# Alexander-H-Liu/End-to-end-ASR-Pytorch

Hardware: NVIDIA H100
Metric: utterances/sec (train step, ~12s@16kHz synthetic) (higher is better)
Workload: dtype f32

## Files before the change

end-to-end-asr-pytorch_b200/csrc/gemm.cu:

```cuda
#include <cuda.h>
#include <cuda_fp16.h>
#include <stdlib.h>
#include "common.cuh"
#include "wgmma.cuh"
#include "../../include/b200asr.h"

namespace b200asr {
namespace {

constexpr int G_BM = 128, G_BN = 128, G_BK = 32;
constexpr int G_TILE = G_BM * G_BK * 4;
constexpr int G_CONSUMERS = 256;
constexpr int G_THREADS = 128 + G_CONSUMERS;
constexpr int G_PREP_WARPS = 3;
constexpr int G_PRODUCER_REGS = 40, G_CONSUMER_REGS = 232;
constexpr int G_BOX = 32 * G_BK * 4;
constexpr int G_MAX_SPLIT = 32;
constexpr int G_CH_DEFAULT = 4;

template <bool B_MN>
struct GemmSmem {
    static constexpr int STAGE = (B_MN ? 4 : 3) * G_TILE;
    static constexpr int STAGES = B_MN ? 3 : 4;
    static constexpr int B_LO = 2 * G_TILE;
// ... 417 lines not shown

struct F16Args {
    const float* bias;
    const float* sa;
    const float* sb;
    float* C;
    float* partial;
    int M, N, ldc, accumulate, perm;
    int KB, kb_per_split;
};

__device__ __forceinline__ int f16_scale_exp(uint32_t amax) {
    if (amax == 0u || amax >= 0x7f800000u) return 0;
    const int E = amax >= 0x00800000u ? (int)(amax >> 23) - 127 : (31 - __clz((int)amax)) - 149;
    return min(126, max(-126, 13 - E));
}
__device__ __forceinline__ float pow2f(int e) { return __uint_as_float((uint32_t)(127 + e) << 23); }
__device__ __forceinline__ uint32_t abs_bits(float x) { return __float_as_uint(x) & 0x7fffffffu; }
__device__ __forceinline__ void f16_split2(float x0, float x1, float s, __half2& hi, __half2& lo) {
    const float y0 = x0 * s, y1 = x1 * s;
    hi = __floats2half2_rn(y0, y1);
    lo = __floats2half2_rn(y0 - __low2float(hi), y1 - __high2float(hi));
}

__global__ void __launch_bounds__(256) f16_split_rows_kernel(const float* __restrict__ x, long long ld, int rows, int K,
                                                             int Kp, __half* __restrict__ hi, __half* __restrict__ lo,
                                                             float* __restrict__ sinv) {
    const int row = blockIdx.x * 8 + (threadIdx.x >> 5), lane = threadIdx.x & 31, c = blockIdx.y;
    if (row >= rows) return;
    const int k = c * F_CK + 4 * lane;
    float4 v = make_float4(0.f, 0.f, 0.f, 0.f);
    if (k < K) v = *reinterpret_cast<const float4*>(x + (size_t)row * ld + k);
    const uint32_t a = __reduce_max_sync(0xffffffffu, max(max(abs_bits(v.x), abs_bits(v.y)), max(abs_bits(v.z), abs_bits(v.w))));
    const int e = f16_scale_exp(a);
    const float s = pow2f(e);
    __half2 h[2], l[2];
    f16_split2(v.x, v.y, s, h[0], l[0]);
    f16_split2(v.z, v.w, s, h[1], l[1]);
    const size_t o = (size_t)row * Kp + k;
    *reinterpret_cast<uint2*>(hi + o) = *reinterpret_cast<const uint2*>(h);
    *reinterpret_cast<uint2*>(lo + o) = *reinterpret_cast<const uint2*>(l);
    if (lane == 0) sinv[(size_t)c * rows + row] = pow2f(-e);
}

__global__ void __launch_bounds__(256) f16_split_cols_kernel(const float* __restrict__ x, long long ld, long long bstride,
                                                             int shift, int T, int R, int cols, int Rp,
                                                             __half* __restrict__ hi, __half* __restrict__ lo,
                                                             float* __restrict__ sinv) {
    __shared__ float tile[F_CK][65];
    const int r0 = blockIdx.y * F_CK, c0 = blockIdx.x * 64, tid = threadIdx.x;
    const int cq = 4 * (tid & 15);
#pragma unroll
    for (int i = 0; i < F_CK / 16; ++i) {
        const int rr = (tid >> 4) + 16 * i, r = r0 + rr;
        float4 v = make_float4(0.f, 0.f, 0.f, 0.f);
        if (r < R && c0 + cq < cols) {
            const int b = r / T, t = r - b * T + shift;
            if (t >= 0 && t < T) v = *reinterpret_cast<const float4*>(x + b * bstride + (long long)t * ld + c0 + cq);
        }
        tile[rr][cq] = v.x; tile[rr][cq + 1] = v.y; tile[rr][cq + 2] = v.z; tile[rr][cq + 3] = v.w;
    }
    __syncthreads();
    const int warp = tid >> 5, lane = tid & 31;
    for (int j = 0; j < 8; ++j) {
        const int cc = 8 * warp + j, col = c0 + cc;
        if (col >= cols) break;
        const float v0 = tile[2 * lane][cc], v1 = tile[2 * lane + 1][cc];
        const float v2 = tile[64 + 2 * lane][cc], v3 = tile[65 + 2 * lane][cc];
        const uint32_t a = __reduce_max_sync(0xffffffffu, max(max(abs_bits(v0), abs_bits(v1)), max(abs_bits(v2), abs_bits(v3))));
        const int e = f16_scale_exp(a);
        const float s = pow2f(e);
        __half2 h0, l0, h1, l1;
        f16_split2(v0, v1, s, h0, l0);
        f16_split2(v2, v3, s, h1, l1);
        const size_t o = (size_t)col * Rp + r0 + 2 * lane;
        *reinterpret_cast<__half2*>(hi + o) = h0;
        *reinterpret_cast<__half2*>(hi + o + 64) = h1;
        *reinterpret_cast<__half2*>(lo + o) = l0;
        *reinterpret_cast<__half2*>(lo + o + 64) = l1;
        if (lane == 0) sinv[(size_t)blockIdx.y * cols + col] = pow2f(-e);
    }
}

__device__ __forceinline__ void f16_chunk(float (&d)[64], int i0, const uint8_t* smem, uint64_t* full, uint64_t* empty,
                                          uint32_t a_off, int lane) {
#pragma unroll
    for (int j = 0; j < F_CH; ++j) {
        const int i = i0 + j, s = i % F_STAGES;
        mbar_wait(&full[s], (uint32_t)((i / F_STAGES) & 1));
        const uint32_t st = smem_u32(smem + s * F_STAGE);
        const uint32_t ahi = st + a_off, alo = ahi + F_TILE, bhi = st + 2 * F_TILE, blo = st + 3 * F_TILE;
        wgmma::fence_operand(d);
        wgmma::fence();
#pragma unroll
        for (int k = 0; k < F_BK / 16; ++k) {
            const uint64_t dah = wgmma::desc_k_sw128(ahi + 32 * k), dbh = wgmma::desc_k_sw128(bhi + 32 * k);
            wgmma::mma_f16_n128(d, dah, dbh, (j | k) != 0);
            wgmma::mma_f16_n128(d, dah, wgmma::desc_k_sw128(blo + 32 * k), 1);
            wgmma::mma_f16_n128(d, wgmma::desc_k_sw128(alo + 32 * k), dbh, 1);
        }
        wgmma::commit_group();
        if (j + 1 < F_CH) wgmma::wait_group<1>();
        else wgmma::wait_all();
        if (lane == 0 && j > 0) g_arrive(&empty[(i - 1) % F_STAGES]);
    }
    wgmma::fence_operand(d);
    if (lane == 0) g_arrive(&empty[(i0 + F_CH - 1) % F_STAGES]);
}

__global__ void __launch_bounds__(G_THREADS, 1)
gemm_f16x3_kernel(const __grid_constant__ CUtensorMap map_ahi, const __grid_constant__ CUtensorMap map_alo,
                  const __grid_constant__ CUtensorMap map_bhi, const __grid_constant__ CUtensorMap map_blo,
                  const F16Args g) {
    extern __shared__ __align__(1024) uint8_t smem[];
    uint64_t* full = reinterpret_cast<uint64_t*>(smem + F_STAGES * F_STAGE);
    uint64_t* empty = full + F_STAGES;
    const int tid = threadIdx.x, warp = tid >> 5, lane = tid & 31;
    const int m0 = blockIdx.y * G_BM, n0 = blockIdx.x * G_BN;
    const int kb0 = blockIdx.z * g.kb_per_split;
    auto slice_blocks = [&]() { return min(g.KB, kb0 + g.kb_per_split) - kb0; };
    if (tid == 0) {
        for (int s = 0; s < F_STAGES; ++s) {
            mbar_init(&full[s], 1);
            mbar_init(&empty[s], G_CONSUMERS / 32);
        }
        mbar_fence_init();
    }
    __syncthreads();

    if (warp < 4) {
        asm volatile("setmaxnreg.dec.sync.aligned.u32 %0;" ::"n"(G_PRODUCER_REGS) : "memory");
        if (warp == 0 && lane == 0) {
            const int nkb = slice_blocks();
            for (int i = 0; i < nkb; ++i) {
                const int s = i % F_STAGES, k = (kb0 + i) * F_BK;
                if (i >= F_STAGES) mbar_wait(&empty[s], (uint32_t)(((i / F_STAGES) - 1) & 1));
                uint8_t* st = smem + s * F_STAGE;
                mbar_expect_tx(&full[s], 4 * F_TILE);
                tma_load_2d(st, &map_ahi, k, m0, &full[s]);
                tma_load_2d(st + F_TILE, &map_alo, k, m0, &full[s]);
                tma_load_2d(st + 2 * F_TILE, &map_bhi, k, n0, &full[s]);
                tma_load_2d(st + 3 * F_TILE, &map_blo, k, n0, &full[s]);
            }
        }
    } else {
        asm volatile("setmaxnreg.inc.sync.aligned.u32 %0;" ::"n"(G_CONSUMER_REGS) : "memory");
        const int nkb = slice_blocks();
        const int wg = (warp >> 2) - 1;
        const int r0 = 64 * wg + 16 * (warp & 3) + (lane >> 2);
        const int row0 = m0 + r0, row1 = row0 + 8;
        const int M = g.M, N = g.N;
        float acc[64], d[64];
#pragma unroll
        for (int e = 0; e < 64; ++e) acc[e] = 0.f;
        for (int i = 0; i < nkb; i += F_CH) {
            const size_t c = (size_t)((kb0 + i) / F_CH);
            const float sa0 = row0 < M ? g.sa[c * M + row0] : 0.f, sa1 = row1 < M ? g.sa[c * M + row1] : 0.f;
            float sb[32];
#pragma unroll
            for (int gq = 0; gq < 16; ++gq) {
                const int n = n0 + 8 * gq + 2 * (lane & 3);
                sb[2 * gq] = n < N ? g.sb[c * N + n] : 0.f;
                sb[2 * gq + 1] = n + 1 < N ? g.sb[c * N + n + 1] : 0.f;
            }
            f16_chunk(d, i, smem, full, empty, (uint32_t)(wg * 64 * 128), lane);
#pragma unroll
// ... 64 lines not shown
}

extern "C" int b200asr_gemm3x_nn(const float* A, int lda, const float* B, int ldb, const float* bias, float* C, int M,
                                 int N, int K, int ldc, int accumulate, void* workspace, size_t workspace_bytes,
                                 b200asr_stream stream) {
    B200_REQUIRE(A && B && C, "gemm3x_nn: null pointer");
    B200_REQUIRE(M > 0 && N > 0 && K > 0, "gemm3x_nn: bad sizes M=%d N=%d K=%d", M, N, K);
    B200_REQUIRE(lda >= K && (lda % 4) == 0 && ldb >= N && (ldb % 4) == 0 && ldc >= N,
                 "gemm3x_nn: row pitches must be multiples of 4 floats (lda %d ldb %d ldc %d)", lda, ldb, ldc);
    B200_REQUIRE(aligned16(A) && aligned16(B), "gemm3x_nn: operands must be 16-byte aligned");
    CUtensorMap ma, mb;
    int rc = make_map_k(&ma, A, M, K, lda, G_BM);
    if (rc != B200_OK) return rc;
    rc = make_map_mn(&mb, B, N, K, 1, ldb, 0, false);
    if (rc != B200_OK) return rc;
    GemmArgs g = {};
    g.bias = bias; g.C = C; g.M = M; g.N = N; g.ldc = ldc; g.accumulate = accumulate;
    g.KB = (K + G_BK - 1) / G_BK; g.kbt = g.KB;
    return launch<false, true>(ma, mb, g, workspace, workspace_bytes, (cudaStream_t)stream);
}

extern "C" int b200asr_gemm3x_nt(const float* A, long long lda, long long a_bstride, int a_shift, const float* B,
                                 long long ldb, long long b_bstride, int b_shift, float* C, int M, int N, int T,
                                 int batches, int ldc, int accumulate, int permute_rows, void* workspace,
                                 size_t workspace_bytes, b200asr_stream stream) {
    B200_REQUIRE(A && B && C, "gemm3x_nt: null pointer");
    B200_REQUIRE(M > 0 && N > 0 && T > 0 && batches > 0, "gemm3x_nt: bad sizes M=%d N=%d T=%d batches=%d", M, N, T,
                 batches);
    B200_REQUIRE(lda > 0 && (lda % 4) == 0 && ldb > 0 && (ldb % 4) == 0 && (a_bstride % 4) == 0 &&
                     (b_bstride % 4) == 0 && ldc >= N,
                 "gemm3x_nt: pitches must be multiples of 4 floats (lda %lld ldb %lld)", lda, ldb);
    B200_REQUIRE(aligned16(A) && aligned16(B), "gemm3x_nt: operands must be 16-byte aligned");
    B200_REQUIRE(!permute_rows || (M % 4) == 0, "gemm3x_nt: the row permutation needs M %% 4 == 0");
    B200_REQUIRE(a_shift >= -G_BK && a_shift <= G_BK && b_shift >= -G_BK && b_shift <= G_BK, "gemm3x_nt: bad shift");
    CUtensorMap ma, mb;
    int rc = make_map_mn(&ma, A, M, T, batches, lda, a_bstride, true);
    if (rc != B200_OK) return rc;
    rc = make_map_mn(&mb, B, N, T, batches, ldb, b_bstride, false);
    if (rc != B200_OK) return rc;
    GemmArgs g = {};
    g.C = C; g.M = M; g.N = N; g.ldc = ldc; g.accumulate = accumulate; g.perm = permute_rows;
    g.kbt = (T + G_BK - 1) / G_BK; g.KB = g.kbt * batches;
    g.a_shift = a_shift; g.b_shift = b_shift;
    return launch<true, true>(ma, mb, g, workspace, workspace_bytes, (cudaStream_t)stream);
}

extern "C" int b200asr_tf32_residual(const float* x, float* lo, long long n, b200asr_stream stream) {
    B200_REQUIRE(x && lo && n >= 0, "tf32_residual: bad arguments");
    if (n == 0) return B200_OK;
    const long long per_block = 256LL * RES_UNROLL * 4;
    tf32_residual_kernel<<<(unsigned)((n + per_block - 1) / per_block), 256, 0, (cudaStream_t)stream>>>(x, lo, n);
    B200_LAUNCH_CHECK("tf32_residual_kernel");
    return B200_OK;
}

extern "C" int b200asr_f16x3_padded_k(int K) { return K > 0 ? (K + F_CK - 1) / F_CK * F_CK : 0; }

extern "C" int b200asr_f16x3_split_rows(const float* x, long long ld, int rows, int K, void* hi, void* lo, float* sinv,
                                        b200asr_stream stream) {
    B200_REQUIRE(x && hi && lo && sinv, "f16x3_split_rows: null pointer");
    B200_REQUIRE(rows > 0 && K > 0 && (K % 4) == 0 && ld >= K && (ld % 4) == 0 && aligned16(x),
                 "f16x3_split_rows: needs K %% 4 == 0, a pitch that is a multiple of 4 floats, 16-byte alignment "
                 "(rows %d K %d ld %lld)", rows, K, ld);
    const int Kp = b200asr_f16x3_padded_k(K);
    dim3 grid((rows + 7) / 8, Kp / F_CK);
    f16_split_rows_kernel<<<grid, 256, 0, (cudaStream_t)stream>>>(x, ld, rows, K, Kp, (__half*)hi, (__half*)lo, sinv);
    B200_LAUNCH_CHECK("f16_split_rows_kernel");
    return B200_OK;
}

extern "C" int b200asr_f16x3_split_cols(const float* x, long long ld, long long bstride, int shift, int T, int batches,
                                        int cols, void* hi, void* lo, float* sinv, b200asr_stream stream) {
    B200_REQUIRE(x && hi && lo && sinv, "f16x3_split_cols: null pointer");
    B200_REQUIRE(T > 0 && batches > 0 && cols > 0 && (cols % 4) == 0 && ld >= cols && (ld % 4) == 0 &&
                     (bstride % 4) == 0 && (batches == 1 || bstride >= (long long)T * ld) && aligned16(x),
                 "f16x3_split_cols: needs cols %% 4 == 0, pitches that are multiples of 4 floats, 16-byte alignment "
                 "(cols %d ld %lld bstride %lld)", cols, ld, bstride);
    B200_REQUIRE((long long)T * batches < (1LL << 31) - F_CK, "f16x3_split_cols: too many rows");
    const int R = T * batches, Rp = b200asr_f16x3_padded_k(R);
    dim3 grid((cols + 63) / 64, Rp / F_CK);
    f16_split_cols_kernel<<<grid, 256, 0, (cudaStream_t)stream>>>(x, ld, bstride, shift, T, R, cols, Rp, (__half*)hi,
                                                                  (__half*)lo, sinv);
    B200_LAUNCH_CHECK("f16_split_cols_kernel");
    return B200_OK;
}

extern "C" int b200asr_gemm_f16x3(const void* a_hi, const void* a_lo, const float* a_sinv, const void* b_hi,
                                  const void* b_lo, const float* b_sinv, const float* bias, float* C, int M, int N,
                                  int Kp, int ldc, int accumulate, int permute_rows, void* workspace,
                                  size_t workspace_bytes, b200asr_stream stream) {
    B200_REQUIRE(a_hi && a_lo && a_sinv && b_hi && b_lo && b_sinv && C, "gemm_f16x3: null pointer");
    B200_REQUIRE(M > 0 && N > 0 && Kp > 0 && (Kp % F_CK) == 0 && ldc >= N,
                 "gemm_f16x3: bad sizes M=%d N=%d Kp=%d ldc=%d (Kp must be b200asr_f16x3_padded_k of K)", M, N, Kp, ldc);
    B200_REQUIRE(aligned16(a_hi) && aligned16(a_lo) && aligned16(b_hi) && aligned16(b_lo),
                 "gemm_f16x3: images must be 16-byte aligned");
    B200_REQUIRE(!permute_rows || (M % 4) == 0, "gemm_f16x3: the row permutation needs M %% 4 == 0");
    CUtensorMap mah, mal, mbh, mbl;
    int rc;
    if ((rc = make_map_f16(&mah, a_hi, M, Kp)) != B200_OK) return rc;
    if ((rc = make_map_f16(&mal, a_lo, M, Kp)) != B200_OK) return rc;
    if ((rc = make_map_f16(&mbh, b_hi, N, Kp)) != B200_OK) return rc;
    if ((rc = make_map_f16(&mbl, b_lo, N, Kp)) != B200_OK) return rc;
    F16Args g = {};
    g.bias = bias; g.sa = a_sinv; g.sb = b_sinv; g.C = C;
    g.M = M; g.N = N; g.ldc = ldc; g.accumulate = accumulate; g.perm = permute_rows;
    g.KB = Kp / F_BK;
    int nsplit = pick_split(M, N, Kp / G_BK);
    if (nsplit > 1 && (workspace == nullptr || workspace_bytes < (size_t)nsplit * M * N * sizeof(float))) nsplit = 1;
    const int chunks = g.KB / F_CH;
    g.kb_per_split = (chunks + nsplit - 1) / nsplit * F_CH;
    nsplit = (g.KB + g.kb_per_split - 1) / g.kb_per_split;
    g.partial = reinterpret_cast<float*>(workspace);
    const size_t smem = (size_t)F_STAGES * F_STAGE + 256;
    cudaStream_t st = (cudaStream_t)stream;
    B200_CUDA(cudaFuncSetAttribute(gemm_f16x3_kernel, cudaFuncAttributeMaxDynamicSharedMemorySize, (int)smem));
    dim3 grid((N + G_BN - 1) / G_BN, (M + G_BM - 1) / G_BM, nsplit);
    gemm_f16x3_kernel<<<grid, G_THREADS, smem, st>>>(mah, mal, mbh, mbl, g);
    B200_LAUNCH_CHECK("gemm_f16x3_kernel");
    if (nsplit > 1) {
        const long long total = (long long)M * N;
        int blocks = (int)((total + 255) / 256);
        if (blocks > 16 * sm_count()) blocks = 16 * sm_count();
        gemm3x_reduce_kernel<<<blocks, 256, 0, st>>>(g.partial, nsplit, bias, C, M, N, ldc, accumulate, permute_rows);
        B200_LAUNCH_CHECK("gemm3x_reduce_kernel");
    }
    return B200_OK;
}
```

end-to-end-asr-pytorch_b200/lib.py:

```python
import ctypes
import os
from ctypes import c_int, c_float, c_longlong, c_size_t, c_void_p, c_char_p, c_ulonglong, POINTER

import torch

_HERE = os.path.dirname(os.path.abspath(__file__))
LIB_PATH = os.path.join(_HERE, "libb200asr.so")

_lib = None

_P = c_void_p
SIGNATURES = {
    "b200asr_version": (c_int, []),
    "b200asr_last_error": (c_char_p, []),
    "b200asr_launch_count": (c_ulonglong, []),
    "b200asr_launch_count_reset": (None, []),
    "b200asr_device_sm_count": (c_int, []),
    "b200asr_fbank_fwd": (c_int, [_P, _P, c_int, c_int, c_int, c_int, c_int, c_float, c_int, _P, c_int, _P, _P, _P, _P,
                                  c_int, c_int, c_float, _P, c_int, _P, _P]),
    "b200asr_fbank_fwd_pcm16": (c_int, [_P, _P, c_int, c_int, c_int, c_int, c_int, c_float, c_int, _P, c_int, _P, _P, _P, _P,
                                  c_int, c_int, c_float, _P, c_int, _P, _P]),
    "b200asr_delta_cmvn_workspace_bytes": (c_size_t, [c_int, c_int, c_int, c_int]),
    "b200asr_delta_cmvn_fwd": (c_int, [_P, _P, c_int, c_int, c_int, c_int, c_int, c_int, c_float, _P, _P, c_size_t,
                                       _P]),
    "b200asr_log_softmax_fwd": (c_int, [_P, _P, _P, _P, c_longlong, c_int, _P]),
    "b200asr_log_softmax_bwd": (c_int, [_P, _P, _P, c_longlong, c_int, _P]),
    "b200asr_ctc_workspace_bytes": (c_size_t, [c_int, c_int, c_int]),
    "b200asr_ctc_fwd_bwd": (c_int, [_P, c_longlong, c_longlong, _P, _P, _P, c_int, c_int, c_int, c_int, c_int, _P, _P,
                                    _P, _P, c_size_t, _P]),
    "b200asr_ctc_grad": (c_int, [_P, c_longlong, c_longlong, _P, _P, _P, c_int, c_int, c_int, c_int, c_int, _P, _P, _P,
                                 _P, _P, c_size_t, _P]),
    "b200asr_ctc_fwd_bwd_logits": (c_int, [_P, _P, c_longlong, c_longlong, _P, _P, _P, c_int, c_int, c_int, c_int, c_int, _P,
                                           _P, _P, _P, c_size_t, _P]),
    "b200asr_ctc_grad_logits": (c_int, [_P, _P, c_longlong, c_longlong, _P, _P, _P, c_int, c_int, c_int, c_int, c_int, _P,
                                        _P, _P, _P, _P, c_size_t, _P]),
    "b200asr_ctc_prefix_score": (c_int, [_P, c_int, c_int, _P, _P, _P, _P, c_int, c_int, c_int, c_int, _P, _P, _P]),
    "b200asr_bilstm_workspace_bytes": (c_size_t, [c_int, c_int, c_int, c_int]),
    "b200asr_bilstm_plan": (c_int, [c_int, c_int, c_int, POINTER(c_int), POINTER(c_int), POINTER(c_int)]),
    "b200asr_bilstm_uses_tensor_cores": (c_int, [c_int, c_int, c_int]),
    "b200asr_bilstm_uses_tcgen05": (c_int, [c_int, c_int, c_int]),
    "b200asr_bilstm_fwd": (c_int, [_P, _P, _P, _P, c_int, c_int, c_int, c_int, _P, c_size_t, _P]),
    "b200asr_bilstm_bwd": (c_int, [_P, _P, _P, _P, c_int, c_int, c_int, c_int, _P, c_size_t, _P]),
    "b200asr_debug_set_lstm_trace": (None, [_P]),
    "b200asr_debug_set_lstm_mode": (None, [c_int]),
    "b200asr_debug_lstm_variant": (c_int, [c_int, c_int, c_int, c_int, POINTER(c_int)]),
    "b200asr_debug_ctc_variant": (c_int, [c_int]),
    "b200asr_debug_locattn_bwd_minb": (c_int, [c_int, c_int, c_int, c_int]),
    "b200asr_lstm_cell_fwd": (c_int, [_P, _P, _P, _P, _P, c_int, c_int, _P]),
    "b200asr_lstm_cell_bwd": (c_int, [_P, _P, _P, _P, _P, _P, _P, c_int, c_int, _P]),
    "b200asr_locattn_cluster_size": (c_int, [c_int, c_int]),
    "b200asr_locattn_wpart_floats": (c_size_t, [c_int, c_int, c_int]),
    "b200asr_locattn_fwd": (c_int, [_P, _P, _P, _P, _P, _P, _P, _P, _P, c_float, c_int, c_int, c_int, c_int, c_int,
                                    c_int, _P, _P, _P]),
    "b200asr_locattn_bwd": (c_int, [_P, _P, _P, _P, _P, _P, _P, _P, c_float, _P, _P, _P, c_int, c_int, c_int, c_int,
                                    c_int, c_int, _P, _P, _P, _P, _P, _P]),
    "b200asr_locattn_bwd_acc": (c_int, [_P, _P, _P, _P, _P, _P, _P, _P, c_float, _P, _P, _P, c_int, c_int, c_int, c_int,
                                        c_int, c_int, _P, _P, _P, _P, _P]),
    "b200asr_attn_dvalue": (c_int, [_P, _P, c_int, c_int, c_int, c_int, _P, c_int, _P]),
    "b200asr_ce_fwd_bwd": (c_int, [_P, _P, c_longlong, c_longlong, c_int, _P, _P, _P, _P]),
    "b200asr_embedding_bwd_workspace_bytes": (c_size_t, [c_int, c_int]),
    "b200asr_embedding_bwd": (c_int, [_P, _P, c_int, c_int, c_int, _P, _P, c_size_t, _P]),
    "b200asr_gemm3x_tn": (c_int, [_P, c_int, _P, _P, _P, _P, c_int, c_int, c_int, c_int, c_int, _P, c_size_t, _P]),
    "b200asr_gemm3x_nn": (c_int, [_P, c_int, _P, c_int, _P, _P, c_int, c_int, c_int, c_int, c_int, _P, c_size_t, _P]),
    "b200asr_gemm3x_workspace_bytes": (c_size_t, [c_int, c_int]),
    "b200asr_gemm3x_nt": (c_int, [_P, c_longlong, c_longlong, c_int, _P, c_longlong, c_longlong, c_int, _P, c_int, c_int,
                                  c_int, c_int, c_int, c_int, c_int, _P, c_size_t, _P]),
    "b200asr_tf32_residual": (c_int, [_P, _P, c_longlong, _P]),
    "b200asr_f16x3_padded_k": (c_int, [c_int]),
    "b200asr_f16x3_split_rows": (c_int, [_P, c_longlong, c_int, c_int, _P, _P, _P, _P]),
    "b200asr_f16x3_split_cols": (c_int, [_P, c_longlong, c_longlong, c_int, c_int, c_int, c_int, _P, _P, _P, _P]),
    "b200asr_gemm_f16x3": (c_int, [_P, _P, _P, _P, _P, _P, _P, _P, c_int, c_int, c_int, c_int, c_int, c_int, _P, c_size_t,
                                   _P]),
    "b200asr_split_tf32": (c_int, [_P, _P, _P, c_longlong, _P]),
    "b200asr_grad_norm_scratch_bytes": (c_size_t, []),
    "b200asr_grad_norm": (c_int, [_P, c_longlong, _P, _P, _P]),
    "b200asr_adadelta_step": (c_int, [_P, _P, _P, _P, c_longlong, c_float, c_float, c_float, c_float, _P, c_float, _P]),
    "b200asr_adam_step": (c_int, [_P, _P, _P, _P, c_longlong, c_float, c_float, c_float, c_float, c_float, c_int, _P,
                                  c_float, _P]),
}


class B200AsrError(RuntimeError):
    pass


def load(build_if_missing=False):
    global _lib
    if _lib is not None:
        return _lib
    if not os.path.exists(LIB_PATH):
        if build_if_missing:
            from . import _build
            _build.build()
        else:
            raise B200AsrError(
                "libb200asr.so is missing (%s): run `python -c 'import __graft_entry__ as g; g.build()'`; "
                "there is no CPU fallback" % LIB_PATH)
    lib = ctypes.CDLL(LIB_PATH)
    for name, (res, args) in SIGNATURES.items():
        fn = getattr(lib, name)
        fn.restype = res
        fn.argtypes = args
    _lib = lib
    return lib


def last_error():
    return load().b200asr_last_error().decode("utf-8", "replace")


def check(rc, what=""):
    if rc != 0:
        raise B200AsrError("%s failed (rc=%d): %s" % (what or "b200asr call", rc, last_error()))


def ptr(t):
    if t is None:
        return None
    if not t.is_cuda:
        raise B200AsrError("b200asr kernels need CUDA tensors (got a %s tensor); there is no CPU fallback" % t.device)
    return c_void_p(t.data_ptr())


def stream():
    return c_void_p(torch.cuda.current_stream().cuda_stream)


def launch_count():
    return int(load().b200asr_launch_count())


def launch_count_reset():
    load().b200asr_launch_count_reset()


class KernelTimer:

    def __init__(self):
        self.enabled = False
        self.records = []

    def reset(self):
        self.records = []

    def summary(self):
        out = {}
        for name, a, b, nbytes in self.records:
            d = out.setdefault(name, {"launches": 0, "ms": 0.0, "bytes": 0})
            d["launches"] += 1
            d["ms"] += a.elapsed_time(b)
            d["bytes"] += nbytes
        return out

# ... 21 lines not shown
```

end-to-end-asr-pytorch_b200/ops.py:

```python
import ctypes
import os

import torch
from torch.autograd import Function

from . import lib as L


def _f32c(t):
    if t.dtype != torch.float32:
        raise L.B200AsrError("b200asr kernels compute in fp32 (got %s)" % t.dtype)
    return t if t.is_contiguous() else t.contiguous()


def _gemm_exact():
    torch.backends.cuda.matmul.allow_tf32 = False
    torch.backends.cudnn.allow_tf32 = False


_gemm_exact()

_perm_cache = {}


# ... 29 lines not shown
    b = _f32c(bias) if bias is not None else None
    ws, ws_bytes = None, 0
    if w_lo is not None or M <= 256:
        ws_bytes = lib.b200asr_gemm3x_workspace_bytes(M, N)
        ws = torch.empty(max(ws_bytes, 16), device=a.device, dtype=torch.uint8)
    with L.timed("gemm3x_tn", 4 * (M * K + N * K + M * N * (2 if accumulate else 1))):
        L.check(lib.b200asr_gemm3x_tn(L.ptr(a), K, L.ptr(w), L.ptr(w_lo), L.ptr(b), L.ptr(out), M, N, K, out.stride(0),
                                      int(bool(accumulate)), L.ptr(ws), ws_bytes, L.stream()), "gemm3x_tn")
    return out


def gemm_tn_ld(a_base, lda, M, K, w, bias=None):
    lib = L.load()
    w = _f32c(w)
    N = w.shape[0]
    out = torch.empty((M, N), device=w.device, dtype=torch.float32)
    b = _f32c(bias) if bias is not None else None
    with L.timed("gemm3x_tn", 4 * (M * lda + N * K + M * N)):
        L.check(lib.b200asr_gemm3x_tn(L.ptr(a_base), lda, L.ptr(w), None, L.ptr(b), L.ptr(out), M, N, K, N, 0, None, 0,
                                      L.stream()), "gemm3x_tn")
    return out


def gemm_nn(a, w, out=None, accumulate=False):
    lib = L.load()
    a, w = _f32c(a), _f32c(w)
    M, K = a.shape
    N = w.shape[1]
    if out is None:
        out = torch.empty((M, N), device=a.device, dtype=torch.float32)
        accumulate = False
    assert out.stride(1) == 1 and out.shape == (M, N)
    ws, ws_bytes = None, 0
    if M <= 256:
        ws_bytes = lib.b200asr_gemm3x_workspace_bytes(M, N)
        ws = torch.empty(max(ws_bytes, 16), device=a.device, dtype=torch.uint8)
    with L.timed("gemm3x_nn", 4 * (M * K + N * K + M * N * (2 if accumulate else 1))):
        L.check(lib.b200asr_gemm3x_nn(L.ptr(a), K, L.ptr(w), N, None, L.ptr(out), M, N, K, out.stride(0),
                                      int(bool(accumulate)), L.ptr(ws), ws_bytes, L.stream()), "gemm3x_nn")
    return out


def gemm_nt(a, b, M, N, T, batches=1, lda=None, a_bstride=0, ldb=None, b_bstride=0, b_shift=0, permute_rows=False,
            out=None, accumulate=False):
    lib = L.load()
    lda = M if lda is None else lda
    ldb = N if ldb is None else ldb
    if out is None:
        out = torch.empty((M, N), device=a.device, dtype=torch.float32)
        accumulate = False
    assert out.is_contiguous() and out.dtype == torch.float32 and out.numel() == M * N
    ws_bytes = lib.b200asr_gemm3x_workspace_bytes(M, N)
    ws = torch.empty(max(ws_bytes, 16), device=a.device, dtype=torch.uint8)
    with L.timed("gemm3x_nt", 4 * (batches * T * (M + N) + M * N * (2 if accumulate else 1))):
        L.check(lib.b200asr_gemm3x_nt(L.ptr(a), lda, a_bstride, 0, L.ptr(b), ldb, b_bstride, b_shift, L.ptr(out), M, N,
                                      T, batches, N, int(bool(accumulate)), int(bool(permute_rows)), L.ptr(ws),
                                      ws_bytes, L.stream()),
                "gemm3x_nt")
    return out


def f16_split(x, rows, K, ld=None):
    lib = L.load()
    ld = K if ld is None else ld
    Kp = lib.b200asr_f16x3_padded_k(K)
    img = torch.empty((2, rows, Kp), device=x.device, dtype=torch.float16)
    sinv = torch.empty((Kp // 128, rows), device=x.device, dtype=torch.float32)
    with L.timed("f16_split", 4 * rows * K + 4 * rows * Kp):
        L.check(lib.b200asr_f16x3_split_rows(L.ptr(x), ld, rows, K, L.ptr(img[0]), L.ptr(img[1]), L.ptr(sinv),
                                             L.stream()), "f16x3_split_rows")
    return img, sinv


def f16_split_t(x, cols, T, batches=1, ld=None, bstride=0, shift=0):
    lib = L.load()
    ld = cols if ld is None else ld
    Rp = lib.b200asr_f16x3_padded_k(batches * T)
    img = torch.empty((2, cols, Rp), device=x.device, dtype=torch.float16)
    sinv = torch.empty((Rp // 128, cols), device=x.device, dtype=torch.float32)
    with L.timed("f16_split", 4 * batches * T * cols + 4 * cols * Rp):
        L.check(lib.b200asr_f16x3_split_cols(L.ptr(x), ld, bstride, shift, T, batches, cols, L.ptr(img[0]),
                                             L.ptr(img[1]), L.ptr(sinv), L.stream()), "f16x3_split_cols")
    return img, sinv


def gemm_f16x3(a, b, bias=None, out=None, accumulate=False, permute_rows=False, name="gemm_f16_tn"):
    lib = L.load()
    (aimg, asinv), (bimg, bsinv) = a, b
    M, Kp = aimg.shape[1], aimg.shape[2]
    N = bimg.shape[1]
    assert bimg.shape[2] == Kp
    if out is None:
        out = torch.empty((M, N), device=aimg.device, dtype=torch.float32)
        accumulate = False
    assert out.dtype == torch.float32 and out.stride(1) == 1 and out.shape == (M, N)
    ws_bytes = lib.b200asr_gemm3x_workspace_bytes(M, N)
    ws = torch.empty(max(ws_bytes, 16), device=aimg.device, dtype=torch.uint8)
    bb = _f32c(bias) if bias is not None else None
    with L.timed(name, 4 * Kp * (M + N) + 4 * M * N * (2 if accumulate else 1)):
        L.check(lib.b200asr_gemm_f16x3(L.ptr(aimg[0]), L.ptr(aimg[1]), L.ptr(asinv), L.ptr(bimg[0]), L.ptr(bimg[1]),
                                       L.ptr(bsinv), L.ptr(bb), L.ptr(out), M, N, Kp, out.stride(0),
                                       int(bool(accumulate)), int(bool(permute_rows)), L.ptr(ws), ws_bytes,
                                       L.stream()), "gemm_f16x3")
    return out


class Conv1dK4S2Fn(Function):

    @staticmethod
    def forward(ctx, x, weight, bias):
        x = _f32c(x)
        B, T, C = x.shape
        O = weight.shape[0]
        Tout = T // 2
        Tp = 2 * (Tout + 1)
        xp = torch.zeros((B, Tp, C), device=x.device, dtype=torch.float32)
        xp[:, 1:T + 1] = x
        wm = weight.detach().permute(0, 2, 1).reshape(O, 4 * C).contiguous()
        M = B * (Tp // 2) - 1
        yf = torch.empty((B * (Tp // 2), O), device=x.device, dtype=torch.float32)
        yf[M:] = 0
        yf[:M] = gemm_tn_ld(xp, 2 * C, M, 4 * C, wm, bias.detach() if bias is not None else None)
        ctx.save_for_backward(xp, wm)
        ctx.dims = (B, T, C, O, Tout, Tp, M)
        ctx.has_bias = bias is not None
        return yf.view(B, Tp // 2, O)[:, :Tout]

    @staticmethod
    def backward(ctx, dy):
        xp, wm = ctx.saved_tensors
        B, T, C, O, Tout, Tp, M = ctx.dims
        half = Tp // 2
        dyf = torch.zeros((B, half, O), device=dy.device, dtype=torch.float32)
        dyf[:, :Tout] = dy
        dy2 = dyf.view(B * half, O)
        dx = None
        if ctx.needs_input_grad[0]:
            dcols = gemm_nn(dy2, wm).view(B, half, 2, 2 * C)
            dxp = torch.zeros((B, half + 1, 2 * C), device=dy.device, dtype=torch.float32)
            dxp[:, :half] += dcols[:, :, 0]
            dxp[:, 1:] += dcols[:, :, 1]
            dx = dxp.view(B, Tp + 2, C)[:, 1:T + 1].contiguous()
        dw = db = None
        if ctx.needs_input_grad[1]:
            dwm = gemm_nt(dy2, xp, O, 4 * C, M, ldb=2 * C)
            dw = dwm.view(O, 4, C).permute(0, 2, 1).contiguous()
        if ctx.has_bias and ctx.needs_input_grad[2]:
            db = dy.reshape(-1, O).sum(0)
        return dx, dw, db


def conv1d_k4s2p1(x, conv):
    C = x.shape[-1]
    if (x.is_cuda and conv.kernel_size == (4,) and conv.stride == (2,) and conv.padding == (1,) and x.shape[1] >= 2
            and (2 * C) % 4 == 0):
        return Conv1dK4S2Fn.apply(x, conv.weight, conv.bias)
    return conv(x.transpose(1, 2)).transpose(1, 2)


class Split:

    def __init__(self, x):
        lib = L.load()
        x = _f32c(x)
        self.hi = torch.empty_like(x)
        self.lo = torch.empty_like(x)
# ... 22 lines not shown
        if accumulate:
            out.addmm_(a.lo, b.hi)
        elif bias is not None:
            torch.addmm(bias, a.lo, b.hi, out=out)
        else:
            torch.mm(a.lo, b.hi, out=out)
        out.addmm_(a.hi, b.lo)
        out.addmm_(a.hi, b.hi)
    finally:
        torch.backends.cuda.matmul.allow_tf32 = prev
    return out


class BiLSTMFn(Function):

    @staticmethod
    def forward(ctx, x, ndir, *params):
        lib = L.load()
        sink = None
        if params and isinstance(params[-1], CStateSink):
            sink, params = params[-1], params[:-1]
        assert len(params) == 4 * ndir
        x = _f32c(x)
        B, T, I = x.shape
        H = params[1].shape[1]
        dev = x.device
        ws_bytes = lib.b200asr_bilstm_workspace_bytes(B, T, H, ndir)
        if ws_bytes == 0:
            raise L.B200AsrError("bilstm: no feasible decomposition for B=%d H=%d (H must be a multiple of 16)" % (B, H))
        perm = gate_perm(H, dev)
        f16 = I % 4 == 0
        xo = f16_split(x.view(B * T, I), B * T, I) if f16 else Split(x.view(B * T, I))
        gates = torch.empty((ndir, B, T, H, 4), device=dev, dtype=torch.float32)
        w_ih_p = []
        for d in range(ndir):
            w_ih, w_hh, b_ih, b_hh = params[4 * d:4 * d + 4]
            wp = w_ih.detach().index_select(0, perm)
            bp = (b_ih.detach() + b_hh.detach()).index_select(0, perm)
            if f16:
                gemm_f16x3(xo, f16_split(wp, 4 * H, I), bias=bp, out=gates[d].view(B * T, 4 * H))
            else:
                mm3(xo, Split(wp).t(), out=gates[d].view(B * T, 4 * H), bias=bp)
            w_ih_p.append(wp)
        del xo
        w_hh = torch.stack([_f32c(params[4 * d + 1].detach()) for d in range(ndir)]).contiguous()
        cst = torch.empty((ndir, B, T, H), device=dev, dtype=torch.float32)
        out = torch.empty((B, T, ndir * H), device=dev, dtype=torch.float32)
        ws = torch.empty(ws_bytes, device=dev, dtype=torch.uint8)
        with L.timed("bilstm_fwd", ndir * (24 * B * H * T + 16 * H * H)):
            L.check(lib.b200asr_bilstm_fwd(L.ptr(gates), L.ptr(w_hh), L.ptr(cst), L.ptr(out), B, T, H, ndir,
                                           L.ptr(ws), ws_bytes, L.stream()), "bilstm_fwd")
        if sink is not None:
            sink.cstate = cst
        ctx.ndir = ndir
        ctx.dims = (B, T, I, H)
        ctx.tail = (None,) if sink is not None else ()
        ctx.consumed = False
        ctx.save_for_backward(x, gates, cst, out, w_hh, *w_ih_p)
        return out

    @staticmethod
    def backward(ctx, dout):
        lib = L.load()
        if ctx.consumed:
            raise L.B200AsrError("BiLSTMFn.backward ran twice: the gate stash is overwritten in place")
        ctx.consumed = True
        ndir = ctx.ndir
        B, T, I, H = ctx.dims
        x, gates, cst, out, w_hh = ctx.saved_tensors[:5]
        w_ih_p = ctx.saved_tensors[5:5 + ndir]
        dev = x.device
        dout = _f32c(dout)
        ws_bytes = lib.b200asr_bilstm_workspace_bytes(B, T, H, ndir)
        ws = torch.empty(ws_bytes, device=dev, dtype=torch.uint8)
        with L.timed("bilstm_bwd", 2 * ndir * (24 * B * H * T + 16 * H * H)):
            L.check(lib.b200asr_bilstm_bwd(L.ptr(gates), L.ptr(w_hh), L.ptr(cst), L.ptr(dout), B, T, H, ndir,
                                           L.ptr(ws), ws_bytes, L.stream()), "bilstm_bwd")
        perm = gate_perm(H, dev)
        need_dx = ctx.needs_input_grad[0]
        dx2 = torch.empty((B * T, I), device=dev, dtype=torch.float32) if need_dx else None
        f16 = I % 4 == 0
        if f16:
            xt = f16_split_t(x, I, B * T)
        else:
            xs = Split(x.view(B * T, I))
        grads = []
        for d in range(ndir):
            g2 = gates[d].view(B * T, 4 * H)
            hd = out[:, :, d * H:(d + 1) * H]
            if f16:
                if need_dx:
                    gemm_f16x3(f16_split(g2, B * T, 4 * H), f16_split(w_ih_p[d].t().contiguous(), I, 4 * H), out=dx2,
                               accumulate=(d > 0))
                gt = f16_split_t(g2, 4 * H, B * T)
                dw_ih = gemm_f16x3(gt, xt, permute_rows=True, name="gemm_f16_nt")
                ht = f16_split_t(hd, H, T, batches=B, ld=ndir * H, bstride=T * ndir * H, shift=(-1 if d == 0 else 1))
                dw_hh = gemm_f16x3(gt, ht, permute_rows=True, name="gemm_f16_nt")
                del gt, ht
            else:
                dG = Split(g2)
                if need_dx:
                    mm3(dG, Split(w_ih_p[d]), out=dx2, accumulate=(d > 0))
                dw_ih = torch.empty((4 * H, I), device=dev, dtype=torch.float32)
                dw_ih.index_copy_(0, perm, mm3(dG.t(), xs))
                hprev = torch.zeros((B, T, H), device=dev, dtype=torch.float32)
                if T > 1:
                    if d == 0:
                        hprev[:, 1:] = hd[:, :-1]
                    else:
                        hprev[:, :-1] = hd[:, 1:]
                dw_hh = torch.empty((4 * H, H), device=dev, dtype=torch.float32)
                dw_hh.index_copy_(0, perm, mm3(dG.t(), Split(hprev.view(B * T, H))))
                del dG, hprev
            db = torch.empty((4 * H,), device=dev, dtype=torch.float32)
            db.index_copy_(0, perm, g2.sum(0))
            grads += [dw_ih, dw_hh, db, db.clone()]
        return (dx2.view(B, T, I) if need_dx else None, None, *grads, *ctx.tail)


class CStateSink:
    cstate = None


def bilstm(x, lstm_params, ndir, sink=None):
    return BiLSTMFn.apply(x, ndir, *lstm_params, *((sink,) if sink is not None else ()))


class LogSoftmaxFn(Function):

    @staticmethod
    def forward(ctx, logits, ctc_head=False):
        lib = L.load()
        x = _f32c(logits)
        V = x.shape[-1]
        n = x.numel() // V
        y = torch.empty_like(x)
        am = torch.empty(x.shape[:-1], device=x.device, dtype=torch.int64)
        with L.timed("log_softmax_fwd", 8 * n * V):
            L.check(lib.b200asr_log_softmax_fwd(L.ptr(x), L.ptr(y), None, L.ptr(am), n, V, L.stream()),
                    "log_softmax_fwd")
        ctx.ctc_head = bool(ctc_head)
        ctx.save_for_backward(y)
        ctx.mark_non_differentiable(am)
        return y, am

    @staticmethod
    def backward(ctx, g, _gam):
        (y,) = ctx.saved_tensors
        if ctx.ctc_head and not _CHECK_CTC_HEAD:
            return g, None
        lib = L.load()
        g = _f32c(g)
        V = y.shape[-1]
        n = y.numel() // V
        dx = torch.empty_like(y)
        with L.timed("log_softmax_bwd", 12 * n * V):
            L.check(lib.b200asr_log_softmax_bwd(L.ptr(y), L.ptr(g), L.ptr(dx), n, V, L.stream()), "log_softmax_bwd")
        if ctx.ctc_head:
            err = float((dx - g).abs().max()) / max(float(g.abs().max()), 1e-30)
            if err > 1e-4:
                raise L.B200AsrError("log_softmax(ctc_head=True): upstream gradient is not a CTC gradient "
                                     "(identity-backward error %.2e)" % err)
        return dx, None


_CHECK_CTC_HEAD = os.environ.get("B200ASR_CHECK_CTC_HEAD", "0") == "1"


def log_softmax(logits, ctc_head=False):
    return LogSoftmaxFn.apply(logits, ctc_head)


class CTCHeadOutput:

    def __init__(self, logits, lse, ids, time_major=False):
        self.logits, self.lse, self.ids, self.time_major = logits, lse, ids, time_major

    @property
    def shape(self):
        s = self.logits.shape
        return torch.Size((s[1], s[0], s[2])) if self.time_major else s

    @property
    def device(self):
        return self.logits.device

    def transpose(self, a, b):
        if {a % 3, b % 3} != {0, 1}:
            raise L.B200AsrError("CTCHeadOutput only swaps batch and time")
        return CTCHeadOutput(self.logits, self.lse, self.ids, not self.time_major)

    def argmax(self, dim=-1):
        if dim not in (-1, 2):
            raise L.B200AsrError("CTCHeadOutput.argmax is over the classes")
        return self.ids.transpose(0, 1) if self.time_major else self.ids

    def detach(self):
        return CTCHeadOutput(self.logits.detach(), self.lse, self.ids, self.time_major)
# ... 554 lines not shown
```

include/b200asr.h:

```cpp
#ifndef B200ASR_H
#define B200ASR_H

#include <stddef.h>

#define B200ASR_VERSION 100

#ifdef __cplusplus
extern "C" {
#endif

#if defined(__GNUC__)
#define B200ASR_API __attribute__((visibility("default")))
#else
#define B200ASR_API
#endif

typedef void* b200asr_stream;

B200ASR_API int b200asr_version(void);
B200ASR_API const char* b200asr_last_error(void);
B200ASR_API unsigned long long b200asr_launch_count(void);
B200ASR_API void b200asr_launch_count_reset(void);
B200ASR_API int b200asr_device_sm_count(void);

// ... 32 lines not shown
                               const long long* targets, const long long* input_lengths,
                               const long long* target_lengths, int B, int T, int V, int L_max, int blank, float* nll,
                               const float* grad_scale, float* grad, void* workspace, size_t workspace_bytes,
                               b200asr_stream stream);
B200ASR_API int b200asr_ctc_grad_logits(const float* logits, const float* row_lse, long long stride_b, long long stride_t,
                            const long long* targets, const long long* input_lengths, const long long* target_lengths,
                            int B, int T, int V, int L_max, int blank, const float* nll, const float* grad_scale,
                            const float* upstream, float* grad, void* workspace, size_t workspace_bytes,
                            b200asr_stream stream);

B200ASR_API int b200asr_ctc_prefix_score(const float* log_probs, int T, int V, const float* r_prev, const int* last_char,
                             const int* prefix_len, const int* candidates, int N, int C, int blank, int eos,
                             float* psi, float* r_out, b200asr_stream stream);

B200ASR_API size_t b200asr_bilstm_workspace_bytes(int B, int T, int H, int ndir);
B200ASR_API int b200asr_bilstm_plan(int B, int H, int ndir, int* unit_block, int* batch_block, int* n_ctas);
B200ASR_API int b200asr_bilstm_uses_tensor_cores(int B, int H, int ndir);
B200ASR_API int b200asr_bilstm_uses_tcgen05(int B, int H, int ndir);
B200ASR_API int b200asr_bilstm_fwd(float* gates, const float* w_hh, float* cstate, float* out, int B, int T, int H, int ndir,
                       void* workspace, size_t workspace_bytes, b200asr_stream stream);
B200ASR_API int b200asr_bilstm_bwd(float* gates, const float* w_hh, const float* cstate, const float* dout, int B, int T,
                       int H, int ndir, void* workspace, size_t workspace_bytes, b200asr_stream stream);


B200ASR_API int b200asr_lstm_cell_fwd(const float* preact, const float* c_prev, float* gates, float* c, float* h, int B,
                          int H, b200asr_stream stream);
B200ASR_API int b200asr_lstm_cell_bwd(const float* gates, const float* c_prev, const float* c, const float* dh,
                          const float* dc_next , float* dpreact, float* dc_prev, int B, int H,
                          b200asr_stream stream);

B200ASR_API int b200asr_locattn_cluster_size(int T, int E);
B200ASR_API size_t b200asr_locattn_wpart_floats(int D, int K, int R);
B200ASR_API int b200asr_locattn_fwd(const float* q, const float* key, const float* value, const float* prev_att,
                                    const long long* enc_len, const float* w_conv, const float* w_proj,
                                    const float* w_energy, const float* b_energy, float temperature, int B, int T,
                                    int D, int E, int K, int R, float* attn, float* ctx, b200asr_stream stream);
B200ASR_API int b200asr_locattn_bwd(const float* q, const float* key, const float* value, const float* prev_att,
                                    const long long* enc_len, const float* w_conv, const float* w_proj,
                                    const float* w_energy, float temperature, const float* attn, const float* dctx,
                                    const float* dattn, int B, int T, int D, int E, int K, int R, float* dq_part,
                                    float* dkey, float* dvalue, float* dprev, float* wpart, b200asr_stream stream);
B200ASR_API int b200asr_locattn_bwd_acc(const float* q, const float* key, const float* value, const float* prev_att,
                                        const long long* enc_len, const float* w_conv, const float* w_proj,
                                        const float* w_energy, float temperature, const float* attn, const float* dctx,
                                        const float* dattn, int B, int T, int D, int E, int K, int R, float* dq_part,
                                        float* dkey_acc, float* dprev, float* wpart_acc, b200asr_stream stream);
B200ASR_API int b200asr_attn_dvalue(const float* attn_steps, const float* dctx_steps, int B, int L, int T, int E,
                                    float* dvalue, int accumulate, b200asr_stream stream);

B200ASR_API int b200asr_ce_fwd_bwd(const float* logits, const long long* target, long long ignore_index,
                                   long long n_rows, int V, const float* grad_scale, float* row_loss,
                                   float* dlogits, b200asr_stream stream);

B200ASR_API size_t b200asr_embedding_bwd_workspace_bytes(int N, int V);
B200ASR_API int b200asr_embedding_bwd(const long long* ids, const float* dY, int N, int V, int E, float* dW,
                                      void* workspace, size_t workspace_bytes, b200asr_stream stream);

B200ASR_API size_t b200asr_grad_norm_scratch_bytes(void);
B200ASR_API int b200asr_grad_norm(const float* grad, long long n, float* norm_out, void* scratch, b200asr_stream stream);
B200ASR_API int b200asr_adadelta_step(float* param, const float* grad, float* square_avg, float* acc_delta, long long n,
                          float lr, float rho, float eps, float weight_decay, const float* grad_norm,
                          float max_norm, b200asr_stream stream);
B200ASR_API int b200asr_adam_step(float* param, const float* grad, float* exp_avg, float* exp_avg_sq, long long n, float lr,
                      float beta1, float beta2, float eps, float weight_decay, int step, const float* grad_norm,
                      float max_norm, b200asr_stream stream);

B200ASR_API int b200asr_gemm3x_tn(const float* A, int lda, const float* B, const float* B_lo, const float* bias, float* C,
                      int M, int N, int K, int ldc, int accumulate, void* workspace, size_t workspace_bytes,
                      b200asr_stream stream);
B200ASR_API int b200asr_gemm3x_nn(const float* A, int lda, const float* B, int ldb, const float* bias, float* C, int M, int N,
                      int K, int ldc, int accumulate, void* workspace, size_t workspace_bytes, b200asr_stream stream);
B200ASR_API size_t b200asr_gemm3x_workspace_bytes(int M, int N);
B200ASR_API int b200asr_gemm3x_nt(const float* A, long long lda, long long a_bstride, int a_shift, const float* B,
                      long long ldb, long long b_bstride, int b_shift, float* C, int M, int N, int T, int batches,
                      int ldc, int accumulate, int permute_rows, void* workspace, size_t workspace_bytes,
                      b200asr_stream stream);
B200ASR_API int b200asr_tf32_residual(const float* x, float* lo, long long n, b200asr_stream stream);

B200ASR_API int b200asr_f16x3_padded_k(int K);
B200ASR_API int b200asr_f16x3_split_rows(const float* x, long long ld, int rows, int K, void* hi, void* lo, float* sinv,
                             b200asr_stream stream);
B200ASR_API int b200asr_f16x3_split_cols(const float* x, long long ld, long long bstride, int shift, int T, int batches,
                             int cols, void* hi, void* lo, float* sinv, b200asr_stream stream);
B200ASR_API int b200asr_gemm_f16x3(const void* a_hi, const void* a_lo, const float* a_sinv, const void* b_hi, const void* b_lo,
                       const float* b_sinv, const float* bias, float* C, int M, int N, int Kp, int ldc, int accumulate,
                       int permute_rows, void* workspace, size_t workspace_bytes, b200asr_stream stream);

B200ASR_API int b200asr_split_tf32(const float* x, float* hi, float* lo, long long n, b200asr_stream stream);

#ifdef __cplusplus
}
#endif
#endif
```

Baseline: 801.8.

## Fuse LSTM gate-gradient splits, transpose and bias sum into one kernel

Adds a kernel that reads the gate gradients for all directions once and writes, in one pass, the transposed f16 hi/lo images, the row images and per-block column sums for the bias gradient. The separate per-direction split, split-transpose and sum passes go away. The per-direction dx GEMMs are folded into a single GEMM over a concatenated K dimension, using a host-built transposed weight stack. This cuts memory passes and launches, at the cost of an extra weight-concatenation copy and a small partial-sum reduction.

```diff
diff --git a/end-to-end-asr-pytorch_b200/csrc/gemm.cu b/end-to-end-asr-pytorch_b200/csrc/gemm.cu
--- a/end-to-end-asr-pytorch_b200/csrc/gemm.cu
+++ b/end-to-end-asr-pytorch_b200/csrc/gemm.cu
@@ -523,6 +523,84 @@
     }
 }
 
+constexpr int DG_PITCH = F_CK + 4;
+constexpr int DG_SMEM = F_CK * DG_PITCH * 4;
+
+__global__ void __launch_bounds__(256, 3) f16_split_dg_kernel(const float* __restrict__ g, int R, int cols, int Kp,
+                                                              int Rp, __half* __restrict__ t_hi,
+                                                              __half* __restrict__ t_lo, float* __restrict__ t_sinv,
+                                                              __half* __restrict__ r_hi, __half* __restrict__ r_lo,
+                                                              float* __restrict__ r_sinv, float* __restrict__ colsum) {
+    extern __shared__ float4 dg_smem[];
+    float* tile = reinterpret_cast<float*>(dg_smem);
+    const int r0 = blockIdx.x * F_CK, c0 = blockIdx.y * F_CK, d = blockIdx.z, ndir = gridDim.z;
+    const int warp = threadIdx.x >> 5, lane = threadIdx.x & 31;
+    const float* gd = g + (size_t)d * R * cols;
+    const int c = c0 + 4 * lane;
+    const size_t ldr = (size_t)ndir * Kp;
+#pragma unroll
+    for (int i0 = 0; i0 < F_CK / 8; i0 += 8) {
+        float4 v[8];
+#pragma unroll
+        for (int i = 0; i < 8; ++i) {
+            const int r = r0 + warp + 8 * (i0 + i);
+            v[i] = make_float4(0.f, 0.f, 0.f, 0.f);
+            if (r < R && c < cols) v[i] = *reinterpret_cast<const float4*>(gd + (size_t)r * cols + c);
+        }
+#pragma unroll
+        for (int i = 0; i < 8; ++i) {
+            const int rr = warp + 8 * (i0 + i), r = r0 + rr;
+            *reinterpret_cast<float4*>(tile + rr * DG_PITCH + 4 * lane) = v[i];
+            if (r_hi != nullptr && r < R) {
+                const uint32_t a = __reduce_max_sync(0xffffffffu, max(max(abs_bits(v[i].x), abs_bits(v[i].y)),
+                                                                      max(abs_bits(v[i].z), abs_bits(v[i].w))));
+                const int e = f16_scale_exp(a);
+                const float s = pow2f(e);
+                __half2 h[2], l[2];
+                f16_split2(v[i].x, v[i].y, s, h[0], l[0]);
+                f16_split2(v[i].z, v[i].w, s, h[1], l[1]);
+                const size_t o = (size_t)r * ldr + (size_t)d * Kp + c;
+                *reinterpret_cast<uint2*>(r_hi + o) = *reinterpret_cast<const uint2*>(h);
+                *reinterpret_cast<uint2*>(r_lo + o) = *reinterpret_cast<const uint2*>(l);
+                if (lane == 0) r_sinv[(size_t)(d * (Kp / F_CK) + blockIdx.y) * R + r] = pow2f(-e);
+            }
+        }
+    }
+    __syncthreads();
+    const size_t t_img = (size_t)d * cols * Rp, t_sc = (size_t)d * (Rp / F_CK) * cols;
+    for (int j = 0; j < F_CK / 32; ++j) {
+        const int cc = 4 * (warp + 8 * j), col0 = c0 + cc;
+        if (col0 >= cols) break;
+        float4 u[4];
+#pragma unroll
+        for (int i = 0; i < 4; ++i) u[i] = *reinterpret_cast<const float4*>(tile + (lane + 32 * i) * DG_PITCH + cc);
+#pragma unroll
+        for (int q = 0; q < 4; ++q) {
+            const float x0 = (&u[0].x)[q], x1 = (&u[1].x)[q], x2 = (&u[2].x)[q], x3 = (&u[3].x)[q];
+            const int col = col0 + q;
+            const uint32_t a = __reduce_max_sync(0xffffffffu, max(max(abs_bits(x0), abs_bits(x1)),
+                                                                  max(abs_bits(x2), abs_bits(x3))));
+            const int e = f16_scale_exp(a);
+            const float s = pow2f(e);
+            __half2 h01, l01, h23, l23;
+            f16_split2(x0, x1, s, h01, l01);
+            f16_split2(x2, x3, s, h23, l23);
+            const size_t o = t_img + (size_t)col * Rp + r0 + lane;
+            t_hi[o] = __low2half(h01); t_hi[o + 32] = __high2half(h01);
+            t_hi[o + 64] = __low2half(h23); t_hi[o + 96] = __high2half(h23);
+            t_lo[o] = __low2half(l01); t_lo[o + 32] = __high2half(l01);
+            t_lo[o + 64] = __low2half(l23); t_lo[o + 96] = __high2half(l23);
+            float sum = (x0 + x1) + (x2 + x3);
+#pragma unroll
+            for (int m = 16; m > 0; m >>= 1) sum += __shfl_xor_sync(0xffffffffu, sum, m);
+            if (lane == 0) {
+                t_sinv[t_sc + (size_t)blockIdx.x * cols + col] = pow2f(-e);
+                colsum[(size_t)blockIdx.x * ndir * cols + (size_t)d * cols + col] = sum;
+            }
+        }
+    }
+}
+
 __device__ __forceinline__ void f16_chunk(float (&d)[64], int i0, const uint8_t* smem, uint64_t* full, uint64_t* empty,
                                           uint32_t a_off, int lane) {
 #pragma unroll
@@ -753,6 +831,26 @@
     f16_split_cols_kernel<<<grid, 256, 0, (cudaStream_t)stream>>>(x, ld, bstride, shift, T, R, cols, Rp, (__half*)hi,
                                                                   (__half*)lo, sinv);
     B200_LAUNCH_CHECK("f16_split_cols_kernel");
+    return B200_OK;
+}
+
+extern "C" int b200asr_f16x3_split_dg(const float* g, int ndir, int rows, int cols, void* t_hi, void* t_lo,
+                                      float* t_sinv, void* r_hi, void* r_lo, float* r_sinv, float* colsum,
+                                      b200asr_stream stream) {
+    B200_REQUIRE(g && t_hi && t_lo && t_sinv && colsum, "f16x3_split_dg: null pointer");
+    B200_REQUIRE((r_hi && r_lo && r_sinv) || (!r_hi && !r_lo && !r_sinv),
+                 "f16x3_split_dg: the row images need all of hi, lo and sinv (or none of them)");
+    B200_REQUIRE((ndir == 1 || ndir == 2) && rows > 0 && cols > 0 && (cols % 4) == 0 && aligned16(g),
+                 "f16x3_split_dg: needs 1 or 2 directions, cols %% 4 == 0, 16-byte alignment (ndir %d rows %d cols %d)",
+                 ndir, rows, cols);
+    B200_REQUIRE(rows < (1 << 30) && cols < (1 << 30) / ndir, "f16x3_split_dg: too many rows or columns");
+    const int Rp = b200asr_f16x3_padded_k(rows), Kp = b200asr_f16x3_padded_k(cols);
+    B200_CUDA(cudaFuncSetAttribute(f16_split_dg_kernel, cudaFuncAttributeMaxDynamicSharedMemorySize, DG_SMEM));
+    dim3 grid(Rp / F_CK, Kp / F_CK, ndir);
+    f16_split_dg_kernel<<<grid, 256, DG_SMEM, (cudaStream_t)stream>>>(g, rows, cols, Kp, Rp, (__half*)t_hi,
+                                                                      (__half*)t_lo, t_sinv, (__half*)r_hi,
+                                                                      (__half*)r_lo, r_sinv, colsum);
+    B200_LAUNCH_CHECK("f16_split_dg_kernel");
     return B200_OK;
 }
 
diff --git a/end-to-end-asr-pytorch_b200/lib.py b/end-to-end-asr-pytorch_b200/lib.py
--- a/end-to-end-asr-pytorch_b200/lib.py
+++ b/end-to-end-asr-pytorch_b200/lib.py
@@ -69,6 +69,7 @@
     "b200asr_f16x3_padded_k": (c_int, [c_int]),
     "b200asr_f16x3_split_rows": (c_int, [_P, c_longlong, c_int, c_int, _P, _P, _P, _P]),
     "b200asr_f16x3_split_cols": (c_int, [_P, c_longlong, c_longlong, c_int, c_int, c_int, c_int, _P, _P, _P, _P]),
+    "b200asr_f16x3_split_dg": (c_int, [_P, c_int, c_int, c_int, _P, _P, _P, _P, _P, _P, _P, _P]),
     "b200asr_gemm_f16x3": (c_int, [_P, _P, _P, _P, _P, _P, _P, _P, c_int, c_int, c_int, c_int, c_int, c_int, _P, c_size_t,
                                    _P]),
     "b200asr_split_tf32": (c_int, [_P, _P, _P, c_longlong, _P]),
diff --git a/end-to-end-asr-pytorch_b200/ops.py b/end-to-end-asr-pytorch_b200/ops.py
--- a/end-to-end-asr-pytorch_b200/ops.py
+++ b/end-to-end-asr-pytorch_b200/ops.py
@@ -135,6 +135,36 @@
         L.check(lib.b200asr_f16x3_split_cols(L.ptr(x), ld, bstride, shift, T, batches, cols, L.ptr(img[0]),
                                              L.ptr(img[1]), L.ptr(sinv), L.stream()), "f16x3_split_cols")
     return img, sinv
+
+
+def f16_split_dg(g, row_images=True):
+    lib = L.load()
+    assert g.is_contiguous() and g.dim() == 3
+    ndir, R, C = g.shape
+    Rp, Kp = lib.b200asr_f16x3_padded_k(R), lib.b200asr_f16x3_padded_k(C)
+    timg = torch.empty((2, ndir, C, Rp), device=g.device, dtype=torch.float16)
+    tsinv = torch.empty((ndir, Rp // 128, C), device=g.device, dtype=torch.float32)
+    rimg = rsinv = None
+    if row_images:
+        rimg = torch.empty((2, R, ndir * Kp), device=g.device, dtype=torch.float16)
+        rsinv = torch.empty((ndir * Kp // 128, R), device=g.device, dtype=torch.float32)
+    part = torch.empty((Rp // 128, ndir * C), device=g.device, dtype=torch.float32)
+    nbytes = 4 * ndir * (R * C + C * Rp + (R * Kp if row_images else 0)) + 4 * part.numel()
+    with L.timed("f16_split_dg", nbytes):
+        L.check(lib.b200asr_f16x3_split_dg(L.ptr(g), ndir, R, C, L.ptr(timg[0]), L.ptr(timg[1]), L.ptr(tsinv),
+                                           L.ptr(rimg[0] if row_images else None),
+                                           L.ptr(rimg[1] if row_images else None), L.ptr(rsinv), L.ptr(part),
+                                           L.stream()), "f16x3_split_dg")
+    return ([(timg[:, d], tsinv[d]) for d in range(ndir)], (rimg, rsinv) if row_images else None,
+            part.sum(0).view(ndir, C))
+
+
+def f16_split_cat_t(ws, Kp):
+    C, N = ws[0].shape
+    wt = torch.zeros((N, len(ws), Kp), device=ws[0].device, dtype=torch.float32)
+    for d, w in enumerate(ws):
+        wt[:, d, :C] = w.t()
+    return f16_split(wt.view(N, len(ws) * Kp), N, len(ws) * Kp)
 
 
 def gemm_f16x3(a, b, bias=None, out=None, accumulate=False, permute_rows=False, name="gemm_f16_tn"):
@@ -323,6 +353,10 @@
         f16 = I % 4 == 0
         if f16:
             xt = f16_split_t(x, I, B * T)
+            gts, grow, gsum = f16_split_dg(gates.view(ndir, B * T, 4 * H), row_images=need_dx)
+            if need_dx:
+                gemm_f16x3(grow, f16_split_cat_t(w_ih_p, grow[0].shape[2] // ndir), out=dx2)
+                del grow
         else:
             xs = Split(x.view(B * T, I))
         grads = []
@@ -330,10 +364,7 @@
             g2 = gates[d].view(B * T, 4 * H)
             hd = out[:, :, d * H:(d + 1) * H]
             if f16:
-                if need_dx:
-                    gemm_f16x3(f16_split(g2, B * T, 4 * H), f16_split(w_ih_p[d].t().contiguous(), I, 4 * H), out=dx2,
-                               accumulate=(d > 0))
-                gt = f16_split_t(g2, 4 * H, B * T)
+                gt = gts[d]
                 dw_ih = gemm_f16x3(gt, xt, permute_rows=True, name="gemm_f16_nt")
                 ht = f16_split_t(hd, H, T, batches=B, ld=ndir * H, bstride=T * ndir * H, shift=(-1 if d == 0 else 1))
                 dw_hh = gemm_f16x3(gt, ht, permute_rows=True, name="gemm_f16_nt")
@@ -354,7 +385,7 @@
                 dw_hh.index_copy_(0, perm, mm3(dG.t(), Split(hprev.view(B * T, H))))
                 del dG, hprev
             db = torch.empty((4 * H,), device=dev, dtype=torch.float32)
-            db.index_copy_(0, perm, g2.sum(0))
+            db.index_copy_(0, perm, gsum[d] if f16 else g2.sum(0))
             grads += [dw_ih, dw_hh, db, db.clone()]
         return (dx2.view(B, T, I) if need_dx else None, None, *grads, *ctx.tail)
 
diff --git a/include/b200asr.h b/include/b200asr.h
--- a/include/b200asr.h
+++ b/include/b200asr.h
@@ -138,6 +138,8 @@
                              b200asr_stream stream);
 B200ASR_API int b200asr_f16x3_split_cols(const float* x, long long ld, long long bstride, int shift, int T, int batches,
                              int cols, void* hi, void* lo, float* sinv, b200asr_stream stream);
+B200ASR_API int b200asr_f16x3_split_dg(const float* g, int ndir, int rows, int cols, void* t_hi, void* t_lo, float* t_sinv,
+                           void* r_hi, void* r_lo, float* r_sinv, float* colsum, b200asr_stream stream);
 B200ASR_API int b200asr_gemm_f16x3(const void* a_hi, const void* a_lo, const float* a_sinv, const void* b_hi, const void* b_lo,
                        const float* b_sinv, const float* bias, float* C, int M, int N, int Kp, int ldc, int accumulate,
                        int permute_rows, void* workspace, size_t workspace_bytes, b200asr_stream stream);
```

New measurement: 830.2, median of 6. +3.5%, better.
